# antoyang/TubeDETR

Measured on AMD Instinct MI355X. Metric: training clips/sec (fwd+bwd) at T=100 k=4 res=352, 1/2/4/8 MI355X, higher is better.
Workload: dtype bf16

## Files before the change

### include/tubedetr_hip.h

```cpp
#ifndef TUBEDETR_HIP_H
#define TUBEDETR_HIP_H
#include <stddef.h>
#include <stdint.h>
#ifdef __cplusplus
extern "C" {
#endif

#define TD_F32 0
#define TD_BF16 1
#define TD_U8 2
#define TD_OK 0
#define TD_ERR_INVALID (-1)
#define TD_ERR_LAUNCH (-2)

typedef void* td_stream_t;

const char* td_last_error(void);
int td_abi_version(void);

int td_set_deterministic(int on);
int td_get_deterministic(void);


#define TD_PROF_GEMM_128x128 0
// ... 68 lines not shown
  td_conv_desc d;
  int ldg;
  int ci_real;
  float* dbias;
  int accumulate;
  int prezeroed;
} td_wgrad_job;
size_t td_conv_wgrad_batch_table_bytes(int n_jobs);
int td_conv_wgrad_batch(const td_wgrad_job* jobs, int n_jobs, int dtype, void* table_host, void* table_dev, size_t table_bytes,
                        td_stream_t stream);

typedef struct td_frame_source {
  const void* data;
  int dtype;
  int n;
  const int* index;
  const int* valid_hw;
} td_frame_source;
int td_frames_to_nhwc(const td_frame_source* srcs, int n_srcs, int C, int H, int W, int Cpad, const float* mean,
                      const float* inv_std, void* y, int dtype, td_stream_t stream);

size_t td_resnet_fwd_ws_bytes(int N, int H, int W, const int* nblocks, int dtype, int save);
int td_resnet_num_convs(const int* nblocks);
int td_resnet_fwd(const td_frame_source* srcs, int n_srcs, const float* mean, const float* inv_std, int N, int H, int W,
                  const int* nblocks, const void* const* w_fwd, const float* const* bias, int save, void* ws, size_t ws_bytes,
                  void** feat, int* feat_hw, int stem_pairs, int first_train_stage, int dtype, td_stream_t stream);
int td_bottleneck_fused(const void* x, void* out, const void* w1, const float* b1, const void* w2, const float* b2, const void* w3,
                        const float* b3, const void* wd, const float* bd, int N, int H, int W, int Cin, int dtype, td_stream_t stream);
int td_pw_chain2(const void* y2, const void* w3, const float* b3, const void* residual, void* out, const void* w1, const float* b1,
                 void* h1, int M, int planes, int dtype, td_stream_t stream);
int td_stem_pair_weights(const void* w_fwd_8, void* w_pairs, int Co, int dtype, td_stream_t stream);
int td_stem_pool(const void* x_pairs, const void* w_pairs, const float* bias, void* pooled, int N, int H, int W, int dtype,
                 td_stream_t stream);
size_t td_resnet_bwd_ws_bytes(int N, int H, int W, const int* nblocks, int first_train_stage, int dtype);
size_t td_resnet_bwd_table_bytes(const int* nblocks, int first_train_stage);
int td_resnet_bwd(const void* dfeat, int N, int N_fwd, int H, int W, const int* nblocks, int first_train_stage,
                  const void* const* w_dgrad, const float* const* scale, float* const* dW, const void* fwd_ws, void* ws,
                  size_t ws_bytes, void* table_host, void* table_dev, size_t table_bytes, int dW_prezeroed, int dtype, int only_stage, td_stream_t stream);

int td_weight_prep(const float* W, const float* bn_w, const float* bn_b, const float* bn_rm, const float* bn_rv,
                   const float* bias, int Co, int Ci, int R, int S, int Cpad, void* w_fwd, void* w_dgrad,
                   float* bias_out, float* scale_out, int dtype, td_stream_t stream);

typedef struct td_prep_item {
  const float* W;
  const float *bn_w, *bn_b, *bn_rm, *bn_rv, *bias;
  void *w_fwd, *w_dgrad;
  float *bias_out, *scale_out;
  int Co, Ci, RS, Cpad, Co_alloc, blk0;
} td_prep_item;
int td_weight_prep_batch(const td_prep_item* items_dev, int n, int total_blocks, int dtype, td_stream_t stream);

int td_wgrad_finalize(const float* dw_k, const float* scale, float* dW, int Co, int Ci, int R, int S, int Cpad,
                      int accumulate, td_stream_t stream);

int td_nchw_to_nhwc(const float* x, void* y, int N, int C, int H, int W, int Cpad, int dtype, td_stream_t stream);
int td_nhwc_to_nchw(const void* x, float* y, int N, int C, int H, int W, int dtype, td_stream_t stream);
int td_cast(const void* x, void* y, size_t n, int src_dtype, int dst_dtype, td_stream_t stream);

int td_maxpool3x3s2(const void* x, void* y, int N, int H, int W, int C, int dtype, td_stream_t stream);

int td_add_layernorm_fwd(const void* x, const void* r, const float* gamma, const float* beta, void* y, void* s_out,
                         float* mean, float* rstd, int rows, int cols, float eps, int dtype, td_stream_t stream);
int td_add_layernorm_bwd(const void* dy, const void* s, const float* mean, const float* rstd, const float* gamma,
                         const void* extra, void* ds, float* dgamma, float* dbeta, int rows, int cols, int dtype,
                         td_stream_t stream);
// ... 99 lines not shown
```

### tubedetr_amd/_hip.py

```python
from __future__ import annotations

import ctypes as C
import os

import torch

TD_F32, TD_BF16 = 0, 1
EXPECTED_ABI = 11
_LIB_PATH = os.environ.get("TD_HIP_LIB") or os.path.join(os.path.dirname(os.path.abspath(__file__)), "lib", "libtubedetr_hip.so")
_lib = None


class ConvDesc(C.Structure):
    _fields_ = [(n, C.c_int) for n in ("N", "Hs", "Ws", "C", "Ho", "Wo", "R", "S", "stride", "pad", "mode", "Nc", "ldc", "out_sp", "out_H", "out_W",
                                       "aniso", "stride_w", "pad_w")]


class PrepItem(C.Structure):
    _fields_ = [(n, C.c_void_p) for n in ("W", "bn_w", "bn_b", "bn_rm", "bn_rv", "bias", "w_fwd", "w_dgrad", "bias_out", "scale_out")] + \
               [(n, C.c_int) for n in ("Co", "Ci", "RS", "Cpad", "Co_alloc", "blk0")]


class WgradJob(C.Structure):
    _fields_ = [("g", C.c_void_p), ("src", C.c_void_p), ("dW", C.c_void_p), ("scale", C.c_void_p), ("d", ConvDesc), ("ldg", C.c_int), ("ci_real", C.c_int), ("dbias", C.c_void_p), ("accumulate", C.c_int), ("prezeroed", C.c_int)]
# ... 21 lines not shown


class Epilogue(C.Structure):
    _fields_ = [
        ("bias", C.c_void_p),
        ("residual", C.c_void_p),
        ("mask_src", C.c_void_p),
        ("relu", C.c_int),
        ("sigmoid", C.c_int),
        ("dropout_p", C.c_float),
        ("dropout_seed", C.c_uint32),
        ("alpha", C.c_float),
        ("dropout_counter", C.c_void_p),
    ]


_P, _I, _F, _U32, _SZ = C.c_void_p, C.c_int, C.c_float, C.c_uint32, C.c_size_t
_SIGS = {
    "td_prof_enable": [_I],
    "td_prof_dump": [C.c_char_p],
    "td_debug_set_stamp_buffer": [_P],
    "td_prof_collect": [_I, _I, C.POINTER(C.c_longlong), C.POINTER(C.c_double), C.POINTER(C.c_double)],
    "td_prof_collect_bytes": [_I, _I, C.POINTER(C.c_double)],
    "td_conv_gemm": [_P, _P, _P, C.POINTER(ConvDesc), C.POINTER(Epilogue), _I, _P],
    "td_conv_wgrad": [_P, _P, _P, C.POINTER(ConvDesc), _I, _I, _I, _P],
    "td_conv_wgrad_bias": [_P, _P, _P, _P, C.POINTER(ConvDesc), _I, _I, _I, _P],
    "td_conv_wgrad_batch": [C.POINTER(WgradJob), _I, _I, _P, _P, _SZ, _P],
    "td_resnet_num_convs": [C.POINTER(C.c_int)],
    "td_resnet_fwd": [C.POINTER(FrameSource), _I, C.POINTER(C.c_float), C.POINTER(C.c_float), _I, _I, _I, C.POINTER(C.c_int), C.POINTER(_P), C.POINTER(_P), _I, _P, _SZ,
                      C.POINTER(_P), C.POINTER(C.c_int), _I, _I, _I, _P],
    "td_bottleneck_fused": [_P, _P, _P, _P, _P, _P, _P, _P, _P, _P, _I, _I, _I, _I, _I, _P],
    "td_stem_pair_weights": [_P, _P, _I, _I, _P],
    "td_stem_pool": [_P, _P, _P, _P, _I, _I, _I, _I, _P],
    "td_pw_chain2": [_P, _P, _P, _P, _P, _P, _P, _P, _I, _I, _I, _P],
    "td_set_deterministic": [_I],
    "td_get_deterministic": [],
    "td_frames_to_nhwc": [C.POINTER(FrameSource), _I, _I, _I, _I, _I, C.POINTER(C.c_float), C.POINTER(C.c_float), _P, _I, _P],
    "td_resnet_bwd": [_P, _I, _I, _I, _I, C.POINTER(C.c_int), _I, C.POINTER(_P), C.POINTER(_P), C.POINTER(_P), _P, _P, _SZ, _P, _P, _SZ, _I, _I, _I, _P],
    "td_weight_prep_batch": [_P, _I, _I, _I, _P],
    "td_weight_prep": [_P, _P, _P, _P, _P, _P, _I, _I, _I, _I, _I, _P, _P, _P, _P, _I, _P],
    "td_wgrad_finalize": [_P, _P, _P, _I, _I, _I, _I, _I, _I, _P],
    "td_nchw_to_nhwc": [_P, _P, _I, _I, _I, _I, _I, _I, _P],
    "td_nhwc_to_nchw": [_P, _P, _I, _I, _I, _I, _I, _P],
    "td_cast": [_P, _P, _SZ, _I, _I, _P],
    "td_maxpool3x3s2": [_P, _P, _I, _I, _I, _I, _I, _P],
    "td_add_layernorm_fwd": [_P, _P, _P, _P, _P, _P, _P, _P, _I, _I, _F, _I, _P],
    "td_add_layernorm_bwd": [_P, _P, _P, _P, _P, _P, _P, _P, _P, _I, _I, _I, _P],
    "td_colsum": [_P, _P, _I, _I, _I, _I, _P],
    "td_add": [_P, _P, _P, _SZ, _I, _P],
    "td_relu_bwd": [_P, _P, _P, _SZ, _F, _I, _P],
    "td_gelu_fwd": [_P, _P, _SZ, _I, _P],
    "td_gelu_bwd": [_P, _P, _P, _SZ, _I, _P],
    "td_dropout": [_P, _P, _SZ, _F, _U32, _P, _I, _P],
    "td_pos_sine": [_P, _P, _I, _I, _I, _I, _F, _I, _I, _P],
    "td_linear_ex": [_P, _P, _P, _P, C.POINTER(LinearExDesc), C.POINTER(Epilogue), _I, _P],
    "td_rows_copy": [_P, _P, _P, _P, _P, _I, _I, _I, _I, _I, _I, _P],
    "td_rows_segment_sum": [_P, _P, _P, _P, _P, _I, _I, _I, _I, _I, _P],
    "td_criterion_fwd": [_P, _P, _P, _P, _P, _P, _P, _P, _P, _F, _F, _I, _I, _I, _I, _P, _P, _P, _P, _P, _P],
    "td_criterion_bwd": [_P, _P, _P, _P, _P, _P, _P, _P, _I, _I, _I, _P],
    "td_sted_decode": [_P, _P, _I, _I, _P],
    "td_grad_norm_clip": [_P, _SZ, C.POINTER(OptimSegment), _I, _F, _P, _SZ, _P, _P, _P],
    "td_adamw_ema_step": [_P, _P, _P, _P, _P, _SZ, C.POINTER(OptimSegment), _I, _P, _P, _P, _F, _F, _F, _F, _F, _P],
    "td_mha_fwd": [_P, _P, _P, _P, _P, _P, _P, _I, _I, _I, _I, _I, _I, _I, _I, _I, _F, _F, _U32, _P, _I, _P],
    "td_mha_bwd": [_P, _P, _P, _P, _P, _P, _P, _P, _P, _P, _I, _I, _I, _I, _I, _I, _I, _I, _I, _F, _F, _U32, _P, _I, _P],
    "td_cross_q1_fwd": [_P, _P, _P, _P, _P, _P, _P, _I, _I, _I, _I, _I, _F, _U32, _P, _I, _P],
    "td_cross_q1_bwd": [_P, _P, _P, _P, _P, _P, _P, _P, _I, _I, _I, _I, _I, _I, _F, _U32, _P, _I, _P],
# ... 76 lines not shown
```

### tubedetr_amd/csrc/bottleneck.hip

```cpp
#include <stdlib.h>

#include <algorithm>
#include <type_traits>

#include "td_common.h"

namespace td {

typedef __bf16 bn_bf16x2 __attribute__((ext_vector_type(2)));
__device__ __forceinline__ uint32_t bn_cvt_pk(float lo, float hi) {
  bn_bf16x2 v = {(__bf16)lo, (__bf16)hi};
  return *(uint32_t*)&v;
}
__device__ __forceinline__ uint32_t bn_relu_pk(uint32_t v) {
  uint32_t r;
  asm("v_pk_max_i16 %0, %1, 0" : "=v"(r) : "v"(v));
  return r;
}
__device__ __forceinline__ uint2 bn_relu_pack4(const f32x4& a) { return make_uint2(bn_relu_pk(bn_cvt_pk(a[0], a[1])), bn_relu_pk(bn_cvt_pk(a[2], a[3]))); }
#ifndef TD_BN_XCD_CONTIG
#define TD_BN_XCD_CONTIG 1
#endif
struct BnTile {
  int img, ty, tx;
// ... 3 lines not shown
};
__device__ __forceinline__ BnWalk bn_walk(int n_tiles) {
  const int b = (int)blockIdx.x, g = (int)gridDim.x;
  BnWalk w;
  if ((g & 7) == 0 && TD_BN_XCD_CONTIG) {
    const int x = b & 7, l = b >> 3, per = (n_tiles + 7) >> 3;
    const int lim = min(per, n_tiles - x * per);
    w.stride = g >> 3;
    w.start = x * per + l;
    w.count = lim > l ? (lim - l + w.stride - 1) / w.stride : 0;
  } else {
    w.stride = g;
    w.start = b;
    w.count = b < n_tiles ? (n_tiles - b + g - 1) / g : 0;
  }
  return w;
}
typedef unsigned int bn_u32x2 __attribute__((ext_vector_type(2)));
__device__ __forceinline__ void bn_store8(__amdgpu_buffer_rsrc_t rs, uint32_t off, uint2 v) {
  __builtin_amdgcn_raw_buffer_store_b64(bn_u32x2{v.x, v.y}, rs, (int)off, 0, 0);
}
typedef unsigned int bn_u32x4 __attribute__((ext_vector_type(4)));
__device__ __forceinline__ void bn_store16(__amdgpu_buffer_rsrc_t rs, uint32_t off, uint4 v) {
  __builtin_amdgcn_raw_buffer_store_b128(bn_u32x4{v.x, v.y, v.z, v.w}, rs, (int)off, 0, 0);
}
__device__ __forceinline__ void bn_store16s(__amdgpu_buffer_rsrc_t rs, uint32_t voff, uint32_t soff, uint4 v) {
  __builtin_amdgcn_raw_buffer_store_b128(bn_u32x4{v.x, v.y, v.z, v.w}, rs, (int)voff, (int)soff, 0);
}
__device__ __forceinline__ void bn_lds_store8(char* p, uint2 v) {
  const uint32_t a = (uint32_t)(uintptr_t)(__attribute__((address_space(3))) char*)p;
  asm volatile("ds_write_b64 %0, %1" ::"v"(a), "v"(v) : "memory");
}
#define TD_BN_OOB 0xFFFFFFF0u
#ifndef TD_BN_ABL
#define TD_BN_ABL 0
#endif
#define TD_BN_STAGE_BYTES 2048
#define TD_BN_BARRIER()                                  \
  do {                                                   \
    asm volatile("s_waitcnt lgkmcnt(0)" ::: "memory");   \
    __builtin_amdgcn_s_barrier();                        \
  } while (0)

struct BneckParams {
  const char* x;
  char* out;
  const char* w1;
  const char* w2;
  const char* w3;
  const char* wd;
  const float *b1, *b2, *b3, *bd;
  int N, H, W;
  int tiles_y, tiles_x, n_tiles;
};

__global__ __launch_bounds__(512, 2) void bottleneck_resident3_kernel(BneckParams p) {
  constexpr int CIN = 256, NC = 4;
  constexpr int TH = 8, TW = 8, HW = TW + 2;
  constexpr int HROWS = 112;
  constexpr int NP = 7;
  constexpr int HP = 160;
  constexpr int XBUF = NC * HROWS * 128;
  __shared__ __attribute__((aligned(16))) char xall0[XBUF];
  __shared__ __attribute__((aligned(16))) char xall1[XBUF];
  __shared__ __attribute__((aligned(16))) char h1[HROWS * HP];
  __shared__ __attribute__((aligned(16))) char h2[TH * TW * HP];
// ... 35 lines not shown
  auto advance = [&](BnTile c) {
    c.tx += g_tx;
    const int kx = c.tx >= p.tiles_x ? 1 : 0;
    c.tx -= kx ? p.tiles_x : 0;
    c.ty += g_ty + kx;
    const int ky = c.ty >= p.tiles_y ? 1 : 0;
    c.ty -= ky ? p.tiles_y : 0;
    c.img += g_img + ky;
    return c;
  };
  uint32_t voff[NP];
  {
    const int lrow = lane0 >> 3;
    const uint32_t lane_part = (uint32_t)(cg * 128 + (((lane0 & 7) ^ lrow) << 4));
#pragma unroll
    for (int k = 0; k < NP; ++k) {
      const int row = (half * NP + k) * 8 + lrow;
      const int hy = (row * 205) >> 11, hx = row - hy * HW;
      voff[k] = row < 100 ? (uint32_t)(hy * p.W + hx) * (CIN * 2) + lane_part : TD_BN_OOB;
    }
  }
  uint4 eye = make_uint4(0u, 0u, 0u, 0u);
  if ((lr >> 3) == lg) {
    const uint32_t one = 0x3F80u << (16 * (lr & 1));
    const int d2 = (lr & 7) >> 1;
    eye.x = d2 == 0 ? one : 0u; eye.y = d2 == 1 ? one : 0u; eye.z = d2 == 2 ? one : 0u; eye.w = d2 == 3 ? one : 0u;
  }
  const uint32_t st_lane = (uint32_t)(((lane0 >> 4) * p.W + ((lane0 >> 3) & 1)) * 512 + cg * 128 + (lane0 & 7) * 16);
  auto issue_tile = [&](BnTile c, char* xbuf) {
    const int y0 = c.ty * TH, x0 = c.tx * TW;
    const bool exists = c.img < p.N;
    const bool interior = exists && y0 >= 1 && x0 >= 1 && y0 + TH + 1 <= p.H && x0 + TW + 1 <= p.W;
    const uint32_t px = (uint32_t)((c.img * p.H + y0) * p.W + x0);
    char* dst = xbuf + cg * (HROWS * 128) + half * NP * 1024;
    if (interior) {
      const uint32_t soff = (uint32_t)__builtin_amdgcn_readfirstlane((int)((px - (uint32_t)(p.W + 1)) * (CIN * 2)));
#pragma unroll
      for (int k = 0; k < NP; ++k) {
#if TD_BN_ABL & 1
        asm volatile("" ::"v"(voff[k]), "s"(soff));
#else
        __builtin_amdgcn_raw_ptr_buffer_load_lds(rs_x, (lds_p)(dst + k * 1024), 16, voff[k], soff, 0, 0);
#endif
      }
    } else {
      int ln = lane0;
      asm volatile("" : "+v"(ln));
      const int lrow = ln >> 3;
#pragma unroll
      for (int k = 0; k < NP; ++k) {
        const int row = (half * NP + k) * 8 + lrow;
        const int hy = (row * 205) >> 11, hx = row - hy * HW;
        uint32_t off = (px - (uint32_t)(p.W + 1)) * (CIN * 2) + voff[k];
        const bool ok = row < 100 && exists && (unsigned)(y0 - 1 + hy) < (unsigned)p.H && (unsigned)(x0 - 1 + hx) < (unsigned)p.W;
        off = ok ? off : TD_BN_OOB;
#if TD_BN_ABL & 1
        asm volatile("" ::"v"(off));
#else
        __builtin_amdgcn_raw_ptr_buffer_load_lds(rs_x, (lds_p)(dst + k * 1024), 16, off, 0, 0, 0);
#endif
      }
    }
  };

  auto process = [&](BnTile tc, BnTile tnext, auto B_) {
    constexpr int B = decltype(B_)::value;
    char* const xb_w = B ? xall1 : xall0;
    char* const xo_w = B ? xall0 : xall1;
    int lane = lane0;
    asm volatile("" : "+v"(lane));
    const int lr = lane & 15, lg = lane >> 4;
    const int cyl = lr >> 1, cxl = lr & 1;
    const int y0 = tc.ty * TH, x0 = tc.tx * TW;
    const uint32_t tile_px = (uint32_t)((tc.img * p.H + y0) * p.W + x0);
    const bool interior = y0 >= 1 && x0 >= 1 && y0 + TH + 1 <= p.H && x0 + TW + 1 <= p.W;
    issue_tile(tnext, xo_w);
    asm volatile("s_waitcnt vmcnt(%0)" ::"n"(NP) : "memory");
    TD_BN_BARRIER();
    const char* const xb = xb_w;
    {
      const char* const xa0 = xb + lr * 128 + ((lg ^ (lr & 7)) << 4) + half * (4 * 2048);
      const char* const xa1 = xb + lr * 128 + (((4 + lg) ^ (lr & 7)) << 4) + half * (4 * 2048);
      f32x4 acc[4];
#pragma unroll
      for (int j = 0; j < 4; ++j) acc[j] = f32x4{b1v[0], b1v[1], b1v[2], b1v[3]};
      uint4 fr[2][4];
      auto load_g = [&](int ks8, uint4 (&dst)[4]) {
        const char* base = ((ks8 & 1) ? xa1 : xa0) + (ks8 >> 1) * (HROWS * 128);
#pragma unroll
        for (int j = 0; j < 4; ++j) dst[j] = *(const uint4*)(base + j * 2048);
      };
      load_g(0, fr[0]);
// ... 198 lines not shown
  }

  const BnWalk walk = bn_walk(p.n_tiles);
  if (walk.count <= 0) return;
  const int g_img = walk.stride / tiles_per_img, g_rem = walk.stride - g_img * tiles_per_img;
  const int g_ty = g_rem / p.tiles_x, g_tx = g_rem - g_ty * p.tiles_x;
  auto advance = [&](BnTile c) {
    c.tx += g_tx;
    const int kx = c.tx >= p.tiles_x ? 1 : 0;
    c.tx -= kx ? p.tiles_x : 0;
    c.ty += g_ty + kx;
    const int ky = c.ty >= p.tiles_y ? 1 : 0;
    c.ty -= ky ? p.tiles_y : 0;
    c.img += g_img + ky;
    return c;
  };
  uint32_t voff[NP];
  {
    const int lrow = lane0 >> 3;
    const uint32_t lane_part = (uint32_t)(((lane0 & 7) ^ lrow) << 4);
#pragma unroll
    for (int k = 0; k < NP; ++k) {
      const int row = (wave * NP + k) * 8 + lrow;
      const int hy = (row * 57) >> 10, hx = row - hy * HW;
      voff[k] = row < NHALO ? (uint32_t)(hy * p.W + hx) * (CIN * 2) + lane_part : TD_BN_OOB;
    }
  }
  const uint32_t st_lane = (uint32_t)((lane0 >> 3) * 512 + cg * 128 + (lane0 & 7) * 16);
  auto issue_tile = [&](BnTile c, char* xbuf) {
    const int y0 = c.ty * TH, x0 = c.tx * TW;
    const bool exists = c.img < p.N;
    const bool interior = exists && y0 >= 1 && x0 >= 1 && y0 + TH + 1 <= p.H && x0 + TW + 1 <= p.W;
    const uint32_t px = (uint32_t)((c.img * p.H + y0) * p.W + x0);
    if (interior) {
      const uint32_t soff = (uint32_t)__builtin_amdgcn_readfirstlane((int)((px - (uint32_t)(p.W + 1)) * (CIN * 2)));
#pragma unroll
      for (int k = 0; k < NP; ++k) __builtin_amdgcn_raw_ptr_buffer_load_lds(rs_x, (lds_p)(xbuf + (wave * NP + k) * 1024), 16, voff[k], soff, 0, 0);
    } else {
      int ln = lane0;
      asm volatile("" : "+v"(ln));
      const int lrow = ln >> 3;
#pragma unroll
      for (int k = 0; k < NP; ++k) {
        const int row = (wave * NP + k) * 8 + lrow;
        const int hy = (row * 57) >> 10, hx = row - hy * HW;
        uint32_t off = (px - (uint32_t)(p.W + 1)) * (CIN * 2) + voff[k];
        const bool ok = row < NHALO && exists && (unsigned)(y0 - 1 + hy) < (unsigned)p.H && (unsigned)(x0 - 1 + hx) < (unsigned)p.W;
        off = ok ? off : TD_BN_OOB;
        __builtin_amdgcn_raw_ptr_buffer_load_lds(rs_x, (lds_p)(xbuf + (wave * NP + k) * 1024), 16, off, 0, 0, 0);
      }
    }
  };

  auto process = [&](BnTile tc, BnTile tnext, auto B_) {
    constexpr int B = decltype(B_)::value;
    char* const xb_w = B ? x1buf : x0buf;
    char* const xo_w = B ? x0buf : x1buf;
    int lane = lane0;
    asm volatile("" : "+v"(lane));
    const int lr = lane & 15, lg = lane >> 4;
    const int y0 = tc.ty * TH, x0 = tc.tx * TW;
    const uint32_t tile_px = (uint32_t)((tc.img * p.H + y0) * p.W + x0);
    const bool interior = y0 >= 1 && x0 >= 1 && y0 + TH + 1 <= p.H && x0 + TW + 1 <= p.W;
    issue_tile(tnext, xo_w);
    asm volatile("s_waitcnt vmcnt(%0)" ::"n"(NP) : "memory");
    TD_BN_BARRIER();
    const char* const xb = xb_w;
    {
      const char* const xa0 = xb + (half * 96 + lr) * 128 + ((lg ^ (lr & 7)) << 4);
      const char* const xa1 = xb + (half * 96 + lr) * 128 + (((4 + lg) ^ (lr & 7)) << 4);
      f32x4 acc[6];
#pragma unroll
      for (int j = 0; j < 6; ++j) acc[j] = f32x4{b1v[0], b1v[1], b1v[2], b1v[3]};
      uint4 fr[2][6];
#pragma unroll
      for (int j = 0; j < 6; ++j) {
        fr[0][j] = *(const uint4*)(xa0 + j * 2048);
        fr[1][j] = *(const uint4*)(xa1 + j * 2048);
      }
#pragma unroll
      for (int ks = 0; ks < 2; ++ks)
#pragma unroll
// ... 171 lines not shown
```

### tubedetr_amd/csrc/resnet_exec.hip

```cpp
#include <stdlib.h>

#include <algorithm>
#include <vector>

#include "td_common.h"

namespace td {

struct ConvSpec {
  int cin, cout, k, stride, pad;
};
struct Tens {
  size_t off;
  int H, W, C;
};
struct BlockPlan {
  int conv[4];
  int stride, stage;
  Tens in, h1, h2, idt, out;
};
struct Plan {
  std::vector<ConvSpec> convs;
  std::vector<BlockPlan> blocks;
  Tens x, stem, pool;
// ... 113 lines not shown

}
using namespace td;

extern "C" size_t td_resnet_fwd_ws_bytes(int N, int H, int W, const int* nblocks, int dtype, int save) {
  return make_plan(N, H, W, nblocks, dtype, save).total;
}

extern "C" int td_resnet_num_convs(const int* nblocks) {
  int n = 1;
  for (int s = 0; s < 4; ++s) n += 3 * nblocks[s] + (nblocks[s] > 0 ? 1 : 0);
  return n;
}

extern "C" int td_resnet_fwd(const td_frame_source* srcs, int n_srcs, const float* mean, const float* inv_std, int N, int H, int W,
                             const int* nblocks, const void* const* w_fwd, const float* const* bias, int save, void* ws,
                             size_t ws_bytes, void** feat, int* feat_hw, int stem_pairs, int first_train_stage, int dtype, td_stream_t stream) {
  TD_REQUIRE(srcs && n_srcs >= 1 && nblocks && w_fwd && bias && ws && feat, "td_resnet_fwd: null pointer");
  TD_REQUIRE(dtype == TD_F32 || dtype == TD_BF16, "td_resnet_fwd: bad dtype");
  {
    long long tot = 0;
    for (int i = 0; i < n_srcs; ++i) tot += srcs[i].n;
    TD_REQUIRE(tot == N, "td_resnet_fwd: the sources contribute %lld frames, N = %d", tot, N);
  }
  Plan P = make_plan(N, H, W, nblocks, dtype, save);
  TD_REQUIRE(ws_bytes >= P.total, "td_resnet_fwd: workspace too small (%zu < %zu)", ws_bytes, P.total);
  char* base = (char*)ws;
  int rc;
  const FrameGroups groups(N, H, W, P.es);
  const FrameGroups* fg = save ? nullptr : &groups;
  bool stem_done = false;
  if (stem_pairs) {
    TD_REQUIRE(dtype == TD_BF16 && (W & 1) == 0, "td_resnet_fwd: the pixel-pair stem needs bf16 and an even frame width");
    rc = td_frames_to_nhwc(srcs, n_srcs, 3, H, W, 4, mean, inv_std, base + P.x.off, dtype, stream);
    if (rc) return rc;
    static const int fused = [] { const char* e_ = getenv("TD_STEM_FUSED"); return e_ ? atoi(e_) : 1; }();
    if (fused) {
      rc = td_stem_pool(base + P.x.off, w_fwd[0], bias[0], base + P.pool.off, N, H, W, dtype, stream);
      stem_done = true;
    } else {
      const int step = fg ? fg->step(frame_elems(P.stem)) : N;
      for (int f0 = 0; f0 < N && !rc; f0 += step) {
        td_conv_desc d = {std::min(step, N - f0), H, W / 2, 8, P.stem.H, P.stem.W, 7, 4, 2, 3, 0, 64, 64, 1, 0, 0, 1, 1, 2};
        td_epilogue e;
        memset(&e, 0, sizeof(e));
        e.bias = bias[0];
        e.relu = 1;
        rc = td_conv_gemm(base + P.x.off + (size_t)f0 * H * W * 4 * P.es, w_fwd[0], base + P.stem.off + (size_t)f0 * frame_elems(P.stem) * P.es, &d, &e, dtype, stream);
      }
    }
  } else {
    rc = td_frames_to_nhwc(srcs, n_srcs, 3, H, W, P.x.C, mean, inv_std, base + P.x.off, dtype, stream);
    if (rc) return rc;
    rc = run_conv(base, P.x, P.stem, N, P.convs[0], w_fwd[0], bias[0], nullptr, 1, dtype, stream, fg);
  }
  if (rc) return rc;
  if (!stem_done) {
    const int step = fg ? fg->step(frame_elems(P.stem)) : N;
    for (int f0 = 0; f0 < N; f0 += step)
      if ((rc = td_maxpool3x3s2(base + P.stem.off + (size_t)f0 * frame_elems(P.stem) * P.es, base + P.pool.off + (size_t)f0 * frame_elems(P.pool) * P.es,
                                std::min(step, N - f0), P.stem.H, P.stem.W, 64, dtype, stream)))
        return rc;
  }
  static const int l1_fused = [] { const char* e = getenv("TD_L1_FUSED"); return e ? atoi(e) : 2; }();
  static const int chain_on = [] { const char* e = getenv("TD_CHAIN"); return e ? atoi(e) : 1; }();
  bool h1_done = false;
  for (size_t bi = 0; bi < P.blocks.size(); ++bi) {
    auto& b = P.blocks[bi];
    const int c1 = b.conv[0], c2 = b.conv[1], c3 = b.conv[2], cd = b.conv[3];
    if (l1_fused && (l1_fused >= 2 || cd >= 0) && dtype == TD_BF16 && (!save || b.stage < first_train_stage) && b.stride == 1 && P.convs[c1].cout == 64 &&
// ... 221 lines not shown
```

### tubedetr_amd/csrc/stem.hip

```cpp
#include <stdlib.h>

#include <algorithm>

#include "td_common.h"

namespace td {

typedef __bf16 bf16x2_v __attribute__((ext_vector_type(2)));
typedef unsigned short u16x2_v __attribute__((ext_vector_type(2)));
typedef unsigned int st_u32x4 __attribute__((ext_vector_type(4)));
__device__ __forceinline__ uint32_t cvt_pk_bf16(float lo, float hi) {
  bf16x2_v v = {(__bf16)lo, (__bf16)hi};
  return *(uint32_t*)&v;
}
__device__ __forceinline__ uint32_t relu_pk_bf16(uint32_t v) {
  uint32_t r;
  asm("v_pk_max_i16 %0, %1, 0" : "=v"(r) : "v"(v));
  return r;
}
__device__ __forceinline__ uint32_t max_pk_nonneg_bf16(uint32_t a, uint32_t b) {
  const u16x2_v r = __builtin_elementwise_max(*(const u16x2_v*)&a, *(const u16x2_v*)&b);
  return *(const uint32_t*)&r;
}

#define TD_LDS_BARRIER()                                   \
  do {                                                     \
    asm volatile("s_waitcnt lgkmcnt(0)" ::: "memory");     \
    __builtin_amdgcn_s_barrier();                          \
  } while (0)

struct StemParams {
  const char* x;
  const char* w;
  const float* bias;
  char* y;
  int N, H, WP;
  int CH, CW;
  int PH, PW;
  int tiles_y, tiles_x, n_tiles;
};

template <int TY, int TX>
__global__ __launch_bounds__(256, 2) void stem_pool_kernel(StemParams p) {
  constexpr int CR = 2 * TY + 1, CC = 2 * TX + 1;
  constexpr int MROWS = CR * CC, MB = (MROWS + 15) / 16;
  constexpr int PR = 2 * CR + 5, PC = CC + 3;
  constexpr int CPITCH = 144;
  __shared__ __attribute__((aligned(16))) char patch[PR * PC * 16];
  __shared__ __attribute__((aligned(16))) char ctile[MB * 16 * CPITCH];
  const int t = threadIdx.x;
  const int wave = __builtin_amdgcn_readfirstlane(t >> 6), lane = t & 63;
  const int lr = lane & 15, lg = lane >> 4;
  const __amdgpu_buffer_rsrc_t rs_y = __builtin_amdgcn_make_buffer_rsrc((void*)p.y, 0, (uint32_t)((size_t)p.N * p.PH * p.PW * 128), 0x00020000);
  uint4 wreg[7][4];
#pragma unroll
  for (int r = 0; r < 7; ++r)
#pragma unroll
    for (int i = 0; i < 4; ++i) wreg[r][i] = *(const uint4*)(p.w + ((size_t)(i * 16 + lr) * 224 + r * 32 + lg * 8) * 2);
  float bias4[4][4];
#pragma unroll
  for (int i = 0; i < 4; ++i)
#pragma unroll
    for (int q = 0; q < 4; ++q) bias4[i][q] = p.bias[i * 16 + 4 * lg + q];

  constexpr int PLD = (PR * PC + 255) / 256;
  uint4 pre[PLD];
  auto fetch_patch = [&](int tile) {
    const int img = tile / (p.tiles_y * p.tiles_x);
    const int trem = tile - img * (p.tiles_y * p.tiles_x);
    const int ty = trem / p.tiles_x, tx = trem - ty * p.tiles_x;
    const int iy0 = 2 * (2 * ty * TY - 1) - 3, ix0 = (2 * tx * TX - 1) - 2;
    const char* ximg = p.x + (size_t)img * p.H * p.WP * 16;
#pragma unroll
    for (int j = 0; j < PLD; ++j) {
      const int e = t + j * 256;
      const int r = e / PC, c = e - r * PC;
      const int iy = iy0 + r, ix = ix0 + c;
      pre[j] = make_uint4(0, 0, 0, 0);
      if (e < PR * PC && tile < p.n_tiles && (unsigned)iy < (unsigned)p.H && (unsigned)ix < (unsigned)p.WP)
        pre[j] = *(const uint4*)(ximg + ((size_t)iy * p.WP + ix) * 16);
    }
  };
  auto store_patch = [&]() {
#pragma unroll
    for (int j = 0; j < PLD; ++j) {
      const int e = t + j * 256;
      if (e < PR * PC) *(uint4*)(patch + e * 16) = pre[j];
    }
  };
  fetch_patch(blockIdx.x);
  store_patch();
  for (int tile = blockIdx.x; tile < p.n_tiles; tile += gridDim.x) {
    const int img = tile / (p.tiles_y * p.tiles_x);
    const int trem = tile - img * (p.tiles_y * p.tiles_x);
    const int ty = trem / p.tiles_x, tx = trem - ty * p.tiles_x;
    const int py0 = ty * TY, px0 = tx * TX;
    const int cy0 = 2 * py0 - 1, cx0 = 2 * px0 - 1;
    fetch_patch(tile + gridDim.x);
    TD_LDS_BARRIER();
    for (int mb = wave; mb < MB; mb += 4) {
      const int m = mb * 16 + lr;
      const int mm = m < MROWS ? m : 0;
      const int cyl = mm / CC, cxl = mm - cyl * CC;
      const char* a0 = patch + ((2 * cyl) * PC + cxl + lg) * 16;
      f32x4 acc[4];
#pragma unroll
      for (int i = 0; i < 4; ++i) acc[i] = f32x4{bias4[i][0], bias4[i][1], bias4[i][2], bias4[i][3]};
      uint4 af[7];
#pragma unroll
      for (int r = 0; r < 7; ++r) af[r] = *(const uint4*)(a0 + r * (PC * 16));
#pragma unroll
      for (int r = 0; r < 7; ++r)
#pragma unroll
        for (int i = 0; i < 4; ++i)
          acc[i] = __builtin_amdgcn_mfma_f32_16x16x32_bf16(*(const bf16x8*)&wreg[r][i], *(const bf16x8*)&af[r], acc[i], 0, 0, 0);
      const int cy = cy0 + cyl, cx = cx0 + cxl;
      const bool inside = m < MROWS && (unsigned)cy < (unsigned)p.CH && (unsigned)cx < (unsigned)p.CW;
      const uint32_t keep = inside ? 0xffffffffu : 0u;
#pragma unroll
      for (int i = 0; i < 4; ++i) {
        uint2 o;
        o.x = relu_pk_bf16(cvt_pk_bf16(acc[i][0], acc[i][1])) & keep;
        o.y = relu_pk_bf16(cvt_pk_bf16(acc[i][2], acc[i][3])) & keep;
        *(uint2*)(ctile + m * CPITCH + (i * 16 + 4 * lg) * 2) = o;
      }
    }
    TD_LDS_BARRIER();
#pragma unroll
    for (int it = 0; it < (TY * TX * 8 + 255) / 256; ++it) {
      const int e = t + it * 256;
      const int kq = (e >> 2) & 7;
      const int c8 = ((kq & 2) << 1) + (e & 3);
      const int qe = ((e >> 6) << 3) + (((kq ^ (kq >> 1) ^ (kq >> 2)) & 1) + (kq & 4) + ((e >> 4) & 2));
      const int px_ = qe % TX, py_ = min(qe / TX, TY - 1);
      const int py = py0 + py_, px = px0 + px_;
      uint4 o = make_uint4(0, 0, 0, 0);
#pragma unroll
      for (int dy = 0; dy < 3; ++dy)
#pragma unroll
        for (int dx = 0; dx < 3; ++dx) {
          const uint4 v = *(const uint4*)(ctile + ((2 * py_ + dy) * CC + 2 * px_ + dx) * CPITCH + c8 * 16);
          o.x = max_pk_nonneg_bf16(o.x, v.x);
          o.y = max_pk_nonneg_bf16(o.y, v.y);
          o.z = max_pk_nonneg_bf16(o.z, v.z);
          o.w = max_pk_nonneg_bf16(o.w, v.w);
        }
      const bool live = qe < TY * TX && py < p.PH && px < p.PW;
      const uint32_t off = live ? (uint32_t)((((size_t)img * p.PH + py) * p.PW + px) * 128 + c8 * 16) : 0xFFFFFFF0u;
      __builtin_amdgcn_raw_buffer_store_b128(st_u32x4{o.x, o.y, o.z, o.w}, rs_y, (int)off, 0, 0);
    }
    store_patch();
    TD_LDS_BARRIER();
  }
}

}
using namespace td;

extern "C" int td_stem_pool(const void* x_pairs, const void* w_pairs, const float* bias, void* pooled, int N, int H, int W, int dtype,
                            td_stream_t stream) {
  TD_REQUIRE(x_pairs && w_pairs && bias && pooled, "td_stem_pool: null pointer");
  TD_REQUIRE(dtype == TD_BF16, "td_stem_pool: the fused stem is a bf16 kernel (the exact-fp32 mode runs conv + pool separately)");
  TD_REQUIRE(N >= 1 && H >= 2 && W >= 2 && (W & 1) == 0, "td_stem_pool: frames must have an even width (pixel pairs)");
  StemParams p;
  p.x = (const char*)x_pairs;
  p.w = (const char*)w_pairs;
  p.bias = bias;
  p.y = (char*)pooled;
  p.N = N;
  p.H = H;
  p.WP = W / 2;
  p.CH = (H + 6 - 7) / 2 + 1;
  p.CW = (W + 6 - 7) / 2 + 1;
  p.PH = (p.CH + 2 - 3) / 2 + 1;
  p.PW = (p.CW + 2 - 3) / 2 + 1;
  static const int n_cu = [] {
    int dev = 0, cus = 256;
    if (hipGetDevice(&dev) == hipSuccess) (void)hipDeviceGetAttribute(&cus, hipDeviceAttributeMultiprocessorCount, dev);
    return cus;
  }();
  hipStream_t st = (hipStream_t)stream;
  const bool prof = prof_on();
  if (prof) {
    prof_begin(TD_PROF_FUSED, dtype, 2.0 * N * p.CH * p.CW * 64.0 * 224.0, st, N * p.CH * p.CW, 64, 224, 7, 2, 0);
    prof_set_bytes(((double)N * H * W * 4 + (double)N * p.PH * p.PW * 64 + 64.0 * 224) * 2.0);
  }
  const bool wide = p.PW % 22 == 0;
  const int TX = wide ? 22 : 16, TY = 4;
  p.tiles_y = cdiv(p.PH, TY);
  p.tiles_x = cdiv(p.PW, TX);
  const long long nt = (long long)N * p.tiles_y * p.tiles_x;
  TD_REQUIRE(nt < 2000000000LL && (double)N * p.PH * p.PW * 128.0 < 4294967000.0, "td_stem_pool: pooled tensor exceeds the 4 GiB buffer-descriptor range");
  p.n_tiles = (int)nt;
  static const int per_cu = [] { const char* e = getenv("TD_STEM_WG_PER_CU"); return e ? std::max(1, atoi(e)) : 2; }();
  const int grid = (int)std::min<long long>(nt, (long long)per_cu * n_cu);
  if (wide) stem_pool_kernel<4, 22><<<grid, 256, 0, st>>>(p);
  else stem_pool_kernel<4, 16><<<grid, 256, 0, st>>>(p);
  if (prof) prof_end(st);
  return check_launch("td_stem_pool");
}
```

Measured before the change: 107.4.

## Fuse uint8 frame normalization into the stem conv+pool kernel

Adds a uint8 path to the fused stem kernel that reads raw planar uint8 frames from up to eight sources, normalizes them and converts to bf16 in registers while staging the patch. This removes the separate frames_to_nhwc pass and its bf16 NHWC intermediate write and read. The tile loop is also restructured to step tiles incrementally and precompute per-thread offsets, and the bottleneck LDS DMA destination is hoisted into a scalar register. The cost is scattered 16-bit loads of three channel planes per pixel pair, which may coalesce worse than the old 16-byte loads, plus extra register pressure from frame and source lookups.

```diff
diff --git a/include/tubedetr_hip.h b/include/tubedetr_hip.h
--- a/include/tubedetr_hip.h
+++ b/include/tubedetr_hip.h
@@ -124,6 +124,10 @@
 int td_stem_pair_weights(const void* w_fwd_8, void* w_pairs, int Co, int dtype, td_stream_t stream);
 int td_stem_pool(const void* x_pairs, const void* w_pairs, const float* bias, void* pooled, int N, int H, int W, int dtype,
                  td_stream_t stream);
+#define TD_STEM_U8_MAX_SOURCES 8
+int td_stem_pool_u8_ok(const td_frame_source* srcs, int n_srcs, int W);
+int td_stem_pool_u8(const td_frame_source* srcs, int n_srcs, const float* mean, const float* inv_std, const void* w_pairs,
+                    const float* bias, void* pooled, int N, int H, int W, int dtype, td_stream_t stream);
 size_t td_resnet_bwd_ws_bytes(int N, int H, int W, const int* nblocks, int first_train_stage, int dtype);
 size_t td_resnet_bwd_table_bytes(const int* nblocks, int first_train_stage);
 int td_resnet_bwd(const void* dfeat, int N, int N_fwd, int H, int W, const int* nblocks, int first_train_stage,
diff --git a/tubedetr_amd/_hip.py b/tubedetr_amd/_hip.py
--- a/tubedetr_amd/_hip.py
+++ b/tubedetr_amd/_hip.py
@@ -77,6 +77,8 @@
     "td_bottleneck_fused": [_P, _P, _P, _P, _P, _P, _P, _P, _P, _P, _I, _I, _I, _I, _I, _P],
     "td_stem_pair_weights": [_P, _P, _I, _I, _P],
     "td_stem_pool": [_P, _P, _P, _P, _I, _I, _I, _I, _P],
+    "td_stem_pool_u8_ok": [C.POINTER(FrameSource), _I, _I],
+    "td_stem_pool_u8": [C.POINTER(FrameSource), _I, C.POINTER(C.c_float), C.POINTER(C.c_float), _P, _P, _P, _I, _I, _I, _I, _P],
     "td_pw_chain2": [_P, _P, _P, _P, _P, _P, _P, _P, _I, _I, _I, _P],
     "td_set_deterministic": [_I],
     "td_get_deterministic": [],
diff --git a/tubedetr_amd/csrc/bottleneck.hip b/tubedetr_amd/csrc/bottleneck.hip
--- a/tubedetr_amd/csrc/bottleneck.hip
+++ b/tubedetr_amd/csrc/bottleneck.hip
@@ -59,6 +59,12 @@
   asm volatile("ds_write_b64 %0, %1" ::"v"(a), "v"(v) : "memory");
 }
 #define TD_BN_OOB 0xFFFFFFF0u
+typedef __attribute__((address_space(3))) char* bn_lds_p;
+__device__ __forceinline__ bn_lds_p bn_dma_dst(char* p) {
+  uint32_t a = (uint32_t)(uintptr_t)(bn_lds_p)p;
+  asm volatile("" : "+s"(a));
+  return (bn_lds_p)(uintptr_t)a;
+}
 #ifndef TD_BN_ABL
 #define TD_BN_ABL 0
 #endif
@@ -160,7 +166,7 @@
     const bool exists = c.img < p.N;
     const bool interior = exists && y0 >= 1 && x0 >= 1 && y0 + TH + 1 <= p.H && x0 + TW + 1 <= p.W;
     const uint32_t px = (uint32_t)((c.img * p.H + y0) * p.W + x0);
-    char* dst = xbuf + cg * (HROWS * 128) + half * NP * 1024;
+    const bn_lds_p dst = bn_dma_dst(xbuf + cg * (HROWS * 128) + half * NP * 1024);
     if (interior) {
       const uint32_t soff = (uint32_t)__builtin_amdgcn_readfirstlane((int)((px - (uint32_t)(p.W + 1)) * (CIN * 2)));
 #pragma unroll
@@ -168,7 +174,7 @@
 #if TD_BN_ABL & 1
         asm volatile("" ::"v"(voff[k]), "s"(soff));
 #else
-        __builtin_amdgcn_raw_ptr_buffer_load_lds(rs_x, (lds_p)(dst + k * 1024), 16, voff[k], soff, 0, 0);
+        __builtin_amdgcn_raw_ptr_buffer_load_lds(rs_x, dst + k * 1024, 16, voff[k], soff, 0, 0);
 #endif
       }
     } else {
@@ -185,7 +191,7 @@
 #if TD_BN_ABL & 1
         asm volatile("" ::"v"(off));
 #else
-        __builtin_amdgcn_raw_ptr_buffer_load_lds(rs_x, (lds_p)(dst + k * 1024), 16, off, 0, 0, 0);
+        __builtin_amdgcn_raw_ptr_buffer_load_lds(rs_x, dst + k * 1024, 16, off, 0, 0, 0);
 #endif
       }
     }
@@ -450,10 +456,11 @@
     const bool exists = c.img < p.N;
     const bool interior = exists && y0 >= 1 && x0 >= 1 && y0 + TH + 1 <= p.H && x0 + TW + 1 <= p.W;
     const uint32_t px = (uint32_t)((c.img * p.H + y0) * p.W + x0);
+    const bn_lds_p dst = bn_dma_dst(xbuf + wave * NP * 1024);
     if (interior) {
       const uint32_t soff = (uint32_t)__builtin_amdgcn_readfirstlane((int)((px - (uint32_t)(p.W + 1)) * (CIN * 2)));
 #pragma unroll
-      for (int k = 0; k < NP; ++k) __builtin_amdgcn_raw_ptr_buffer_load_lds(rs_x, (lds_p)(xbuf + (wave * NP + k) * 1024), 16, voff[k], soff, 0, 0);
+      for (int k = 0; k < NP; ++k) __builtin_amdgcn_raw_ptr_buffer_load_lds(rs_x, dst + k * 1024, 16, voff[k], soff, 0, 0);
     } else {
       int ln = lane0;
       asm volatile("" : "+v"(ln));
@@ -465,7 +472,7 @@
         uint32_t off = (px - (uint32_t)(p.W + 1)) * (CIN * 2) + voff[k];
         const bool ok = row < NHALO && exists && (unsigned)(y0 - 1 + hy) < (unsigned)p.H && (unsigned)(x0 - 1 + hx) < (unsigned)p.W;
         off = ok ? off : TD_BN_OOB;
-        __builtin_amdgcn_raw_ptr_buffer_load_lds(rs_x, (lds_p)(xbuf + (wave * NP + k) * 1024), 16, off, 0, 0, 0);
+        __builtin_amdgcn_raw_ptr_buffer_load_lds(rs_x, dst + k * 1024, 16, off, 0, 0, 0);
       }
     }
   };
diff --git a/tubedetr_amd/csrc/resnet_exec.hip b/tubedetr_amd/csrc/resnet_exec.hip
--- a/tubedetr_amd/csrc/resnet_exec.hip
+++ b/tubedetr_amd/csrc/resnet_exec.hip
@@ -169,10 +169,14 @@
   bool stem_done = false;
   if (stem_pairs) {
     TD_REQUIRE(dtype == TD_BF16 && (W & 1) == 0, "td_resnet_fwd: the pixel-pair stem needs bf16 and an even frame width");
-    rc = td_frames_to_nhwc(srcs, n_srcs, 3, H, W, 4, mean, inv_std, base + P.x.off, dtype, stream);
-    if (rc) return rc;
     static const int fused = [] { const char* e_ = getenv("TD_STEM_FUSED"); return e_ ? atoi(e_) : 1; }();
-    if (fused) {
+    static const int stem_u8 = [] { const char* e_ = getenv("TD_STEM_U8"); return e_ ? atoi(e_) : 1; }();
+    if (fused && stem_u8 && td_stem_pool_u8_ok(srcs, n_srcs, W)) {
+      rc = td_stem_pool_u8(srcs, n_srcs, mean, inv_std, w_fwd[0], bias[0], base + P.pool.off, N, H, W, dtype, stream);
+      stem_done = true;
+    } else if ((rc = td_frames_to_nhwc(srcs, n_srcs, 3, H, W, 4, mean, inv_std, base + P.x.off, dtype, stream))) {
+      return rc;
+    } else if (fused) {
       rc = td_stem_pool(base + P.x.off, w_fwd[0], bias[0], base + P.pool.off, N, H, W, dtype, stream);
       stem_done = true;
     } else {
diff --git a/tubedetr_amd/csrc/stem.hip b/tubedetr_amd/csrc/stem.hip
--- a/tubedetr_amd/csrc/stem.hip
+++ b/tubedetr_amd/csrc/stem.hip
@@ -1,3 +1,4 @@
+#include <limits.h>
 #include <stdlib.h>
 
 #include <algorithm>
@@ -38,10 +39,37 @@
   int CH, CW;
   int PH, PW;
   int tiles_y, tiles_x, n_tiles;
-};
-
-template <int TY, int TX>
-__global__ __launch_bounds__(256, 2) void stem_pool_kernel(StemParams p) {
+  int d_img, d_ty, d_tx;
+};
+
+struct StemU8Src {
+  const uint8_t* data;
+  const int* index;
+  const int* valid_hw;
+  int first;
+};
+struct StemU8 {
+  const uint8_t* data[TD_STEM_U8_MAX_SOURCES];
+  const int* index[TD_STEM_U8_MAX_SOURCES];
+  const int* valid_hw[TD_STEM_U8_MAX_SOURCES];
+  int first[TD_STEM_U8_MAX_SOURCES];
+  float mean[3], inv_std[3], in_scale;
+};
+
+struct StemTile {
+  int img, ty, tx;
+};
+struct StemFrame {
+  const uint8_t* planes;
+  int vh, vw;
+};
+
+__device__ __forceinline__ int ld_const(const int* ptr, size_t i) {
+  return ((const __attribute__((address_space(4))) int*)(uintptr_t)ptr)[i];
+}
+
+template <int TY, int TX, bool U8>
+__global__ __launch_bounds__(256, 2) void stem_pool_kernel(StemParams p, StemU8 u) {
   constexpr int CR = 2 * TY + 1, CC = 2 * TX + 1;
   constexpr int MROWS = CR * CC, MB = (MROWS + 15) / 16;
   constexpr int PR = 2 * CR + 5, PC = CC + 3;
@@ -64,39 +92,145 @@
     for (int q = 0; q < 4; ++q) bias4[i][q] = p.bias[i * 16 + 4 * lg + q];
 
   constexpr int PLD = (PR * PC + 255) / 256;
-  uint4 pre[PLD];
-  auto fetch_patch = [&](int tile) {
-    const int img = tile / (p.tiles_y * p.tiles_x);
-    const int trem = tile - img * (p.tiles_y * p.tiles_x);
-    const int ty = trem / p.tiles_x, tx = trem - ty * p.tiles_x;
-    const int iy0 = 2 * (2 * ty * TY - 1) - 3, ix0 = (2 * tx * TX - 1) - 2;
-    const char* ximg = p.x + (size_t)img * p.H * p.WP * 16;
+  int prc[PLD], poff[PLD];
+#pragma unroll
+  for (int j = 0; j < PLD; ++j) {
+    const int e = t + j * 256;
+    const int r = e / PC, c = e - r * PC;
+    prc[j] = (r << 8) | c;
+    poff[j] = U8 ? r * 2 * p.WP + 2 * c : (r * p.WP + c) * 16;
+  }
+  uint4 pre[U8 ? 1 : PLD];
+  uint32_t raw[U8 ? PLD : 1][3];
+  uint32_t pmask = 0;
+  auto tile_of = [&](int tile) {
+    StemTile w;
+    w.img = tile / (p.tiles_y * p.tiles_x);
+    const int trem = tile - w.img * (p.tiles_y * p.tiles_x);
+    w.ty = trem / p.tiles_x;
+    w.tx = trem - w.ty * p.tiles_x;
+    return w;
+  };
+  auto advance = [&](StemTile& w) {
+    w.tx += p.d_tx;
+    if (w.tx >= p.tiles_x) { w.tx -= p.tiles_x; ++w.ty; }
+    w.ty += p.d_ty;
+    if (w.ty >= p.tiles_y) { w.ty -= p.tiles_y; ++w.img; }
+    w.img += p.d_img;
+  };
+  auto frame_src = [&](int img, StemU8Src& s) {
+    int k = 0;
+#pragma unroll
+    for (int i = 1; i < TD_STEM_U8_MAX_SOURCES; ++i) k += img >= u.first[i] ? 1 : 0;
+    s.data = u.data[k];
+    s.index = u.index[k];
+    s.valid_hw = u.valid_hw[k];
+    s.first = u.first[k];
+    if (img >= p.N) return -1;
+    const int local = img - s.first;
+    return s.index ? ld_const(s.index, local) : local;
+  };
+  auto frame_of = [&](const StemU8Src& s, int srcf) {
+    StemFrame f;
+    f.planes = s.data;
+    f.vh = 0;
+    f.vw = 0;
+    if (srcf >= 0) {
+      f.planes += (size_t)srcf * 3 * p.H * (2 * p.WP);
+      f.vh = p.H;
+      f.vw = 2 * p.WP;
+      if (s.valid_hw) {
+        f.vh = min(f.vh, ld_const(s.valid_hw, 2 * (size_t)srcf));
+        f.vw = min(f.vw, ld_const(s.valid_hw, 2 * (size_t)srcf + 1));
+      }
+    }
+    return f;
+  };
+  auto fetch_patch = [&](const StemTile& w, const StemFrame& f) {
+    const int iy0 = 2 * (2 * w.ty * TY - 1) - 3, ix0 = (2 * w.tx * TX - 1) - 2;
+    if constexpr (U8) {
+      const uint32_t plane = (uint32_t)(p.H * (2 * p.WP));
+      const __amdgpu_buffer_rsrc_t rs_x = __builtin_amdgcn_make_buffer_rsrc((void*)f.planes, 0, 3u * plane, 0x00020000);
+      const int o0 = iy0 * (2 * p.WP) + 2 * ix0;
+      pmask = 0;
+#pragma unroll
+      for (int j = 0; j < PLD; ++j) {
+        const int iy = iy0 + (prc[j] >> 8), px = 2 * (ix0 + (prc[j] & 255));
+        const bool row = t + j * 256 < PR * PC && (unsigned)iy < (unsigned)f.vh;
+        const bool in0 = row && (unsigned)px < (unsigned)f.vw, in1 = row && (unsigned)(px + 1) < (unsigned)f.vw;
+        pmask |= ((in0 ? 1u : 0u) | (in1 ? 2u : 0u)) << (2 * j);
+        const int off = in0 ? o0 + poff[j] : (int)0x7FFFFFF0;
+#pragma unroll
+        for (int c = 0; c < 3; ++c) raw[j][c] = (uint16_t)__builtin_amdgcn_raw_buffer_load_b16(rs_x, off, (int)(c * plane), 0);
+      }
+    } else {
+      const char* x0 = p.x + ((size_t)w.img * p.H * p.WP + ((ptrdiff_t)iy0 * p.WP + ix0)) * 16;
+#pragma unroll
+      for (int j = 0; j < PLD; ++j) {
+        const int iy = iy0 + (prc[j] >> 8), ix = ix0 + (prc[j] & 255);
+        pre[j] = make_uint4(0, 0, 0, 0);
+        if (t + j * 256 < PR * PC && w.img < p.N && (unsigned)iy < (unsigned)p.H && (unsigned)ix < (unsigned)p.WP) pre[j] = *(const uint4*)(x0 + poff[j]);
+      }
+    }
+  };
+  auto store_patch = [&]() {
 #pragma unroll
     for (int j = 0; j < PLD; ++j) {
       const int e = t + j * 256;
-      const int r = e / PC, c = e - r * PC;
-      const int iy = iy0 + r, ix = ix0 + c;
-      pre[j] = make_uint4(0, 0, 0, 0);
-      if (e < PR * PC && tile < p.n_tiles && (unsigned)iy < (unsigned)p.H && (unsigned)ix < (unsigned)p.WP)
-        pre[j] = *(const uint4*)(ximg + ((size_t)iy * p.WP + ix) * 16);
-    }
-  };
-  auto store_patch = [&]() {
-#pragma unroll
-    for (int j = 0; j < PLD; ++j) {
-      const int e = t + j * 256;
-      if (e < PR * PC) *(uint4*)(patch + e * 16) = pre[j];
-    }
-  };
-  fetch_patch(blockIdx.x);
+      uint4 v;
+      if constexpr (U8) {
+        uint32_t o[4];
+#pragma unroll
+        for (int k = 0; k < 2; ++k) {
+          float f[3];
+#pragma unroll
+          for (int c = 0; c < 3; ++c)
+            f[c] = __builtin_fmaf((float)((raw[j][c] >> (8 * k)) & 0xffu), u.in_scale, -u.mean[c]) * u.inv_std[c];
+          const uint32_t keep = 0u - ((pmask >> (2 * j + k)) & 1u);
+          o[2 * k] = ((uint32_t)f32_to_bf16(f[0]) | ((uint32_t)f32_to_bf16(f[1]) << 16)) & keep;
+          o[2 * k + 1] = (uint32_t)f32_to_bf16(f[2]) & keep;
+        }
+        v = make_uint4(o[0], o[1], o[2], o[3]);
+      } else {
+        v = pre[j];
+      }
+      if (e < PR * PC) *(uint4*)(patch + e * 16) = v;
+    }
+  };
+  constexpr int PIT = (TY * TX * 8 + 255) / 256;
+  const int kq = (t >> 2) & 7;
+  const int c8 = ((kq & 2) << 1) + (t & 3);
+  int pyx[PIT];
+#pragma unroll
+  for (int it = 0; it < PIT; ++it) {
+    const int e = t + it * 256;
+    const int qe = ((e >> 6) << 3) + (((kq ^ (kq >> 1) ^ (kq >> 2)) & 1) + (kq & 4) + ((e >> 4) & 2));
+    const int px_ = qe % TX, py_ = min(qe / TX, TY - 1);
+    pyx[it] = (py_ << 8) | px_ | (qe < TY * TX ? 1 << 16 : 0);
+  }
+
+  StemTile cur = tile_of(blockIdx.x), nxt = cur;
+  advance(nxt);
+  StemTile nn = nxt;
+  advance(nn);
+  StemFrame f_nxt = {nullptr, 0, 0};
+  if constexpr (U8) {
+    StemU8Src s;
+    const int srcf = frame_src(cur.img, s);
+    fetch_patch(cur, frame_of(s, srcf));
+    const int srcf1 = frame_src(nxt.img, s);
+    f_nxt = frame_of(s, srcf1);
+  } else {
+    fetch_patch(cur, f_nxt);
+  }
   store_patch();
-  for (int tile = blockIdx.x; tile < p.n_tiles; tile += gridDim.x) {
-    const int img = tile / (p.tiles_y * p.tiles_x);
-    const int trem = tile - img * (p.tiles_y * p.tiles_x);
-    const int ty = trem / p.tiles_x, tx = trem - ty * p.tiles_x;
-    const int py0 = ty * TY, px0 = tx * TX;
+  for (; cur.img < p.N;) {
+    const int py0 = cur.ty * TY, px0 = cur.tx * TX;
     const int cy0 = 2 * py0 - 1, cx0 = 2 * px0 - 1;
-    fetch_patch(tile + gridDim.x);
+    StemU8Src s_nn = {nullptr, nullptr, nullptr, 0};
+    int srcf_nn = -1;
+    if constexpr (U8) srcf_nn = frame_src(nn.img, s_nn);
+    fetch_patch(nxt, f_nxt);
     TD_LDS_BARRIER();
     for (int mb = wave; mb < MB; mb += 4) {
       const int m = mb * 16 + lr;
@@ -126,14 +260,12 @@
       }
     }
     TD_LDS_BARRIER();
-#pragma unroll
-    for (int it = 0; it < (TY * TX * 8 + 255) / 256; ++it) {
-      const int e = t + it * 256;
-      const int kq = (e >> 2) & 7;
-      const int c8 = ((kq & 2) << 1) + (e & 3);
-      const int qe = ((e >> 6) << 3) + (((kq ^ (kq >> 1) ^ (kq >> 2)) & 1) + (kq & 4) + ((e >> 4) & 2));
-      const int px_ = qe % TX, py_ = min(qe / TX, TY - 1);
-      const int py = py0 + py_, px = px0 + px_;
+    StemFrame f_nn = {nullptr, 0, 0};
+    if constexpr (U8) f_nn = frame_of(s_nn, srcf_nn);
+    const uint32_t ybase = (uint32_t)((((size_t)cur.img * p.PH + py0) * p.PW + px0) * 128) + c8 * 16;
+#pragma unroll
+    for (int it = 0; it < PIT; ++it) {
+      const int px_ = pyx[it] & 255, py_ = (pyx[it] >> 8) & 255;
       uint4 o = make_uint4(0, 0, 0, 0);
 #pragma unroll
       for (int dy = 0; dy < 3; ++dy)
@@ -145,28 +277,23 @@
           o.z = max_pk_nonneg_bf16(o.z, v.z);
           o.w = max_pk_nonneg_bf16(o.w, v.w);
         }
-      const bool live = qe < TY * TX && py < p.PH && px < p.PW;
-      const uint32_t off = live ? (uint32_t)((((size_t)img * p.PH + py) * p.PW + px) * 128 + c8 * 16) : 0xFFFFFFF0u;
+      const bool live = (pyx[it] >> 16) && py0 + py_ < p.PH && px0 + px_ < p.PW;
+      const uint32_t off = live ? ybase + (uint32_t)((py_ * p.PW + px_) * 128) : 0xFFFFFFF0u;
       __builtin_amdgcn_raw_buffer_store_b128(st_u32x4{o.x, o.y, o.z, o.w}, rs_y, (int)off, 0, 0);
     }
     store_patch();
     TD_LDS_BARRIER();
+    cur = nxt;
+    nxt = nn;
+    f_nxt = f_nn;
+    advance(nn);
   }
 }
 
 }
 using namespace td;
 
-extern "C" int td_stem_pool(const void* x_pairs, const void* w_pairs, const float* bias, void* pooled, int N, int H, int W, int dtype,
-                            td_stream_t stream) {
-  TD_REQUIRE(x_pairs && w_pairs && bias && pooled, "td_stem_pool: null pointer");
-  TD_REQUIRE(dtype == TD_BF16, "td_stem_pool: the fused stem is a bf16 kernel (the exact-fp32 mode runs conv + pool separately)");
-  TD_REQUIRE(N >= 1 && H >= 2 && W >= 2 && (W & 1) == 0, "td_stem_pool: frames must have an even width (pixel pairs)");
-  StemParams p;
-  p.x = (const char*)x_pairs;
-  p.w = (const char*)w_pairs;
-  p.bias = bias;
-  p.y = (char*)pooled;
+static int stem_launch(StemParams& p, const StemU8* u8, int N, int H, int W, int dtype, hipStream_t st, const char* what) {
   p.N = N;
   p.H = H;
   p.WP = W / 2;
@@ -179,23 +306,88 @@
     if (hipGetDevice(&dev) == hipSuccess) (void)hipDeviceGetAttribute(&cus, hipDeviceAttributeMultiprocessorCount, dev);
     return cus;
   }();
-  hipStream_t st = (hipStream_t)stream;
   const bool prof = prof_on();
   if (prof) {
     prof_begin(TD_PROF_FUSED, dtype, 2.0 * N * p.CH * p.CW * 64.0 * 224.0, st, N * p.CH * p.CW, 64, 224, 7, 2, 0);
-    prof_set_bytes(((double)N * H * W * 4 + (double)N * p.PH * p.PW * 64 + 64.0 * 224) * 2.0);
+    prof_set_bytes(u8 ? (double)N * H * W * 3 + ((double)N * p.PH * p.PW * 64 + 64.0 * 224) * 2.0
+                      : ((double)N * H * W * 4 + (double)N * p.PH * p.PW * 64 + 64.0 * 224) * 2.0);
   }
   const bool wide = p.PW % 22 == 0;
   const int TX = wide ? 22 : 16, TY = 4;
   p.tiles_y = cdiv(p.PH, TY);
   p.tiles_x = cdiv(p.PW, TX);
   const long long nt = (long long)N * p.tiles_y * p.tiles_x;
-  TD_REQUIRE(nt < 2000000000LL && (double)N * p.PH * p.PW * 128.0 < 4294967000.0, "td_stem_pool: pooled tensor exceeds the 4 GiB buffer-descriptor range");
+  TD_REQUIRE(nt < 2000000000LL && (double)N * p.PH * p.PW * 128.0 < 4294967000.0, "%s: pooled tensor exceeds the 4 GiB buffer-descriptor range", what);
   p.n_tiles = (int)nt;
   static const int per_cu = [] { const char* e = getenv("TD_STEM_WG_PER_CU"); return e ? std::max(1, atoi(e)) : 2; }();
   const int grid = (int)std::min<long long>(nt, (long long)per_cu * n_cu);
-  if (wide) stem_pool_kernel<4, 22><<<grid, 256, 0, st>>>(p);
-  else stem_pool_kernel<4, 16><<<grid, 256, 0, st>>>(p);
+  p.d_img = grid / (p.tiles_y * p.tiles_x);
+  p.d_ty = (grid - p.d_img * (p.tiles_y * p.tiles_x)) / p.tiles_x;
+  p.d_tx = grid - p.d_img * (p.tiles_y * p.tiles_x) - p.d_ty * p.tiles_x;
+  static const StemU8 none = {};
+  if (u8) {
+    if (wide) stem_pool_kernel<4, 22, true><<<grid, 256, 0, st>>>(p, *u8);
+    else stem_pool_kernel<4, 16, true><<<grid, 256, 0, st>>>(p, *u8);
+  } else {
+    if (wide) stem_pool_kernel<4, 22, false><<<grid, 256, 0, st>>>(p, none);
+    else stem_pool_kernel<4, 16, false><<<grid, 256, 0, st>>>(p, none);
+  }
   if (prof) prof_end(st);
-  return check_launch("td_stem_pool");
-}
+  return check_launch(what);
+}
+
+extern "C" int td_stem_pool(const void* x_pairs, const void* w_pairs, const float* bias, void* pooled, int N, int H, int W, int dtype,
+                            td_stream_t stream) {
+  TD_REQUIRE(x_pairs && w_pairs && bias && pooled, "td_stem_pool: null pointer");
+  TD_REQUIRE(dtype == TD_BF16, "td_stem_pool: the fused stem is a bf16 kernel (the exact-fp32 mode runs conv + pool separately)");
+  TD_REQUIRE(N >= 1 && H >= 2 && W >= 2 && (W & 1) == 0, "td_stem_pool: frames must have an even width (pixel pairs)");
+  StemParams p;
+  p.x = (const char*)x_pairs;
+  p.w = (const char*)w_pairs;
+  p.bias = bias;
+  p.y = (char*)pooled;
+  return stem_launch(p, nullptr, N, H, W, dtype, (hipStream_t)stream, "td_stem_pool");
+}
+
+extern "C" int td_stem_pool_u8_ok(const td_frame_source* srcs, int n_srcs, int W) {
+  if (!srcs || n_srcs < 1 || (W & 1)) return 0;
+  int used = 0;
+  for (int s = 0; s < n_srcs; ++s) {
+    if (srcs[s].n == 0) continue;
+    if (srcs[s].n < 0 || srcs[s].dtype != TD_U8 || !srcs[s].data || ((uintptr_t)srcs[s].data & 1)) return 0;
+    ++used;
+  }
+  return used >= 1 && used <= TD_STEM_U8_MAX_SOURCES;
+}
+
+extern "C" int td_stem_pool_u8(const td_frame_source* srcs, int n_srcs, const float* mean, const float* inv_std, const void* w_pairs,
+                               const float* bias, void* pooled, int N, int H, int W, int dtype, td_stream_t stream) {
+  TD_REQUIRE(srcs && n_srcs >= 1 && w_pairs && bias && pooled, "td_stem_pool_u8: null pointer");
+  TD_REQUIRE(dtype == TD_BF16, "td_stem_pool_u8: the fused stem is a bf16 kernel (the exact-fp32 mode runs conv + pool separately)");
+  TD_REQUIRE(N >= 1 && H >= 2 && W >= 2 && (W & 1) == 0, "td_stem_pool_u8: frames must have an even width (pixel pairs)");
+  TD_REQUIRE(td_stem_pool_u8_ok(srcs, n_srcs, W), "td_stem_pool_u8: needs 1..%d non-empty sources, all of them uint8 pixels at an even address", TD_STEM_U8_MAX_SOURCES);
+  StemU8 u = {};
+  for (int s = 0; s < TD_STEM_U8_MAX_SOURCES; ++s) u.first[s] = INT_MAX;
+  long long tot = 0;
+  int k = 0;
+  for (int s = 0; s < n_srcs; ++s) {
+    if (srcs[s].n == 0) continue;
+    u.data[k] = (const uint8_t*)srcs[s].data;
+    u.index[k] = srcs[s].index;
+    u.valid_hw[k] = srcs[s].valid_hw;
+    u.first[k++] = (int)tot;
+    tot += srcs[s].n;
+  }
+  TD_REQUIRE(tot == N, "td_stem_pool_u8: the sources contribute %lld frames, N = %d", tot, N);
+  for (int c = 0; c < 3; ++c) {
+    u.mean[c] = mean ? mean[c] : 0.f;
+    u.inv_std[c] = inv_std ? inv_std[c] : 1.f;
+  }
+  u.in_scale = 1.f / 255.f;
+  StemParams p;
+  p.x = nullptr;
+  p.w = (const char*)w_pairs;
+  p.bias = bias;
+  p.y = (char*)pooled;
+  return stem_launch(p, &u, N, H, W, dtype, (hipStream_t)stream, "td_stem_pool_u8");
+}
```

New measurement: 107.8, median of 6. No clear change (+0.4%).
